# huawei-noah/Speech-Backbones

Hardware: AMD Instinct MI355X
Metric: mel-frames/sec at N=50 reverse-diffusion, 80x1024 batch (higher is better)
Workload: dtype f32 storage, f16 hi*hi MFMA + fp8 cross-term MFMA (3x3 Block convolutions, Upsample; bf16x3 elsewhere), f32 accumulate; 1 GPU; BASELINE config 2: Grad-TTS LJSpeech decoder, N=50, B=16/GPU synthetic 80x1024 mels, all-ones mask; per_gpu_batch=16, frames=1024, parallelism=utterance-shard x1, weights=seed-0 default init, Rezero.g=0.02, output_finite=True, conv_kernel=conv_ws.hip (persistent, wave-specialised), sub_batch_streams=0, hip_graph=False, launches_per_euler_step=64

## Files before the change

speech-backbones_amd/csrc/attn.hip:

```cpp
#include <cstring>
#include "common.h"
#include "kernels.h"

#ifndef GTTS_ATTN_HPW
#define GTTS_ATTN_HPW 2
#endif

namespace gtts {

struct AttnCtxArgs {
    const void *x;
    const unsigned char *wkv;
    float *partials;
    int C, HW, nstage, tiles, tps, nrec, nsplit, B;
    AttnTail tail;
};

__device__ __forceinline__ void pack8_split(const float (&v)[8], u32x4 &hi, u32x4 &lo) {
    bf16x8 vh, vl;
#pragma unroll
    for (int i = 0; i < 8; ++i) {
        __bf16 h, l;
        split_bf16(v[i], h, l);
        vh[i] = h;
        vl[i] = l;
    }
    hi = *reinterpret_cast<u32x4 *>(&vh);
    lo = *reinterpret_cast<u32x4 *>(&vl);
}

template <int NSPLIT, int FULLC, typename AT = float, int HPW = 1, int TAIL = 0>
__global__ __launch_bounds__(256 * HPW, HPW == 1 ? 2 : 1) void attn_ctx_kernel(const AttnCtxArgs a) {
    constexpr int AB = (int)sizeof(AT);
    static_assert(!TAIL || (FULLC && AB == 4), "the fused tail: whole 32-channel stages, fp32 storage");
    constexpr int KCH = ATTN_KCH, NKG = 2 * KCH;
    constexpr int NKGT = NKG / HPW;
    constexpr int WHEAD = 2 * NKG * 64;
    static_assert(HPW == 1 || HPW == 2, "one or two heads per workgroup");
    constexpr int SM16 = 2 * NKG * 256 + HPW * WHEAD;
    static_assert((size_t)SM16 * 16 >= (size_t)4 * HPW * ATTN_REC * 4, "merge records must fit the staging buffer");
    __shared__ __attribute__((aligned(16))) u32x4 s_all[SM16];
    u32x4 *s_ah = s_all, *s_al = s_all + NKG * 256;
    u32x4 *s_wall = s_all + 2 * NKG * 256;

    const int tid = threadIdx.x, lane = tid & 63;
    const int t255 = tid & 255, hw = __builtin_amdgcn_readfirstlane(tid >> 8);
    const int wave = (tid >> 6) & 3;
    const int l31 = lane & 31, kgl = lane >> 5;
    constexpr int HG = 4 / HPW;
    const int nsl = gridDim.x / (HG * a.B);
    const int wg = xcd_slot(blockIdx.x, gridDim.x);
    const int head = (wg % HG) * HPW + hw, slice = (wg / HG) % nsl, b = (wg / HG) / nsl;
    u32x4 *s_w = s_wall + hw * WHEAD;
    const int tile0 = slice * a.tps;
    const int tile1 = min(tile0 + a.tps, a.tiles);
    const AT *xb = reinterpret_cast<const AT *>(a.x) + (size_t)b * a.C * a.HW;
    const u32x4 *wblk = reinterpret_cast<const u32x4 *>(a.wkv) + (size_t)head * a.nstage * (2 * NKG * 64);

    float raw[NKGT][8];
    u32x4 wregs[KCH];
    const unsigned long long xaddr = reinterpret_cast<unsigned long long>(xb);
    const unsigned xlo = __builtin_amdgcn_readfirstlane((unsigned)xaddr);
    const unsigned xhi = __builtin_amdgcn_readfirstlane((unsigned)(xaddr >> 32));
    const int xbytes = a.C * a.HW * AB;
    const __amdgpu_buffer_rsrc_t rsx = __builtin_amdgcn_make_buffer_rsrc(
        reinterpret_cast<void *>(((unsigned long long)xhi << 32) | xlo), 0, __builtin_amdgcn_readfirstlane(xbytes), 0x00020000);
    [[maybe_unused]] float rawh[NKGT][8], tmask = 0.f;
    [[maybe_unused]] __amdgpu_buffer_rsrc_t rsh = rsx, rsi = rsx;
    [[maybe_unused]] const bool tail_store = (wg % HG) == 0;
    if constexpr (TAIL) {
        auto mk = [&](const void *p) {
            const unsigned long long u = reinterpret_cast<unsigned long long>(reinterpret_cast<const AT *>(p) + (size_t)b * a.C * a.HW);
            const unsigned lo = __builtin_amdgcn_readfirstlane((unsigned)u), hi = __builtin_amdgcn_readfirstlane((unsigned)(u >> 32));
            return __builtin_amdgcn_make_buffer_rsrc(reinterpret_cast<void *>(((unsigned long long)hi << 32) | lo), 0,
                                                     __builtin_amdgcn_readfirstlane(xbytes), 0x00020000);
        };
        rsh = mk(a.tail.h);
        rsi = mk(a.tail.xin);
    }
    auto apply_tail = [&](int tile, int stage) {
        if constexpr (TAIL) {
            const int n = tile * 256 + t255;
            const int voff = n < a.HW ? n * AB : xbytes;
#pragma unroll
            for (int kg = 0; kg < NKGT; ++kg) {
                const int cb = stage * 16 * KCH + (hw * NKGT + kg) * 8;
#pragma unroll
                for (int i = 0; i < 8; ++i) {
                    const float sc = a.tail.esc[(size_t)b * a.C + cb + i], sh = a.tail.esh[(size_t)b * a.C + cb + i];
                    const float v = tail_value(rawh[kg][i], raw[kg][i], sc, sh, tmask);
                    raw[kg][i] = v;
                    if (tail_store) __builtin_amdgcn_raw_buffer_store_b32(__builtin_bit_cast(int, v), rsx, voff, (cb + i) * a.HW * 4, GTTS_OUT_NT);
                }
            }
        }
    };
    auto load = [&](int tile, int stage) {
        const int n = tile * 256 + t255;
        const int voff = n < a.HW ? n * AB : xbytes;
        if constexpr (TAIL) {
            if (stage == 0) tmask = n < a.HW ? a.tail.mask[(size_t)b * a.tail.T + ((size_t)(n % a.tail.W) << a.tail.lvl)] : 0.f;
        }
#pragma unroll
        for (int kg = 0; kg < NKGT; ++kg) {
            const int cb = stage * 16 * KCH + (hw * NKGT + kg) * 8;
#pragma unroll
            for (int i = 0; i < 8; ++i) {
                const int c = FULLC ? cb + i : min(cb + i, a.C - 1);
                float v;
                if constexpr (TAIL) {
                    v = __builtin_bit_cast(float, __builtin_amdgcn_raw_buffer_load_b32(rsi, voff, c * a.HW * 4, 0));
                    rawh[kg][i] = __builtin_bit_cast(float, __builtin_amdgcn_raw_buffer_load_b32(rsh, voff, c * a.HW * 4, 0));
                } else if constexpr (AB == 4) v = __builtin_bit_cast(float, __builtin_amdgcn_raw_buffer_load_b32(rsx, voff, c * a.HW * 4, 0));
                else v = __builtin_bit_cast(float, (unsigned)(unsigned short)__builtin_amdgcn_raw_buffer_load_b16(rsx, voff, c * a.HW * 2, 0) << 16);
                raw[kg][i] = (FULLC || cb + i < a.C) ? v : 0.f;
            }
        }
        const u32x4 *g = wblk + (size_t)stage * (2 * NKG * 64);
#pragma unroll
        for (int j = 0; j < KCH; ++j) wregs[j] = g[t255 + j * 256];
    };

    const float NEG_INF = -__builtin_inff();
    float m_run = NEG_INF, z_run = 0.f;
    f32x16 ctx;
#pragma unroll
    for (int r = 0; r < 16; ++r) ctx[r] = 0.f;
    constexpr bool lo_on = NSPLIT > 1;

    load(tile0, 0);
    for (int tile = tile0; tile < tile1; ++tile) {
        f32x16 acc[2][2];
#pragma unroll
        for (int pf = 0; pf < 2; ++pf)
#pragma unroll
            for (int cf = 0; cf < 2; ++cf)
#pragma unroll
                for (int r = 0; r < 16; ++r) acc[pf][cf][r] = 0.f;

        for (int stage = 0; stage < a.nstage; ++stage) {
            apply_tail(tile, stage);
            lds_barrier();
#pragma unroll
            for (int kg = 0; kg < NKGT; ++kg) {
                u32x4 hi, lo;
                pack8_split(raw[kg], hi, lo);
                s_ah[(hw * NKGT + kg) * 256 + t255] = hi;
                s_al[(hw * NKGT + kg) * 256 + t255] = lo;
            }
#pragma unroll
            for (int j = 0; j < KCH; ++j) s_w[t255 + j * 256] = wregs[j];
            lds_barrier();
            if (stage + 1 < a.nstage) load(tile, stage + 1);
            else if (tile + 1 < tile1) load(tile + 1, 0);
#pragma unroll
            for (int kc = 0; kc < KCH; ++kc) {
                bf16x8 xh[2], xl[2], wh[2], wl[2];
#pragma unroll
                for (int pf = 0; pf < 2; ++pf) {
                    const int xi = (kc * 2 + kgl) * 256 + wave * 64 + pf * 32 + l31;
                    xh[pf] = *reinterpret_cast<const bf16x8 *>(&s_ah[xi]);
                    xl[pf] = *reinterpret_cast<const bf16x8 *>(&s_al[xi]);
                }
#pragma unroll
                for (int cf = 0; cf < 2; ++cf) {
                    const int wi = (kc * 2 + kgl) * 64 + cf * 32 + l31;
                    wh[cf] = *reinterpret_cast<const bf16x8 *>(&s_w[wi]);
                    wl[cf] = *reinterpret_cast<const bf16x8 *>(&s_w[wi + NKG * 64]);
                }
#pragma unroll
                for (int pf = 0; pf < 2; ++pf)
#pragma unroll
                    for (int cf = 0; cf < 2; ++cf) {
                        if (lo_on) {
                            acc[pf][cf] = __builtin_amdgcn_mfma_f32_32x32x16_bf16(xl[pf], wh[cf], acc[pf][cf], 0, 0, 0);
                            acc[pf][cf] = __builtin_amdgcn_mfma_f32_32x32x16_bf16(xh[pf], wl[cf], acc[pf][cf], 0, 0, 0);
                        }
                        acc[pf][cf] = __builtin_amdgcn_mfma_f32_32x32x16_bf16(xh[pf], wh[cf], acc[pf][cf], 0, 0, 0);
                    }
            }
        }

        const int nbase = tile * 256 + wave * 64 + 4 * kgl;
        const bool full = tile * 256 + 256 <= a.HW;
        float tmax = NEG_INF;
        if (full) {
#pragma unroll
            for (int pf = 0; pf < 2; ++pf)
#pragma unroll
                for (int rg = 0; rg < 16; ++rg) tmax = fmaxf(tmax, acc[pf][0][rg]);
        } else {
#pragma unroll
            for (int pf = 0; pf < 2; ++pf)
#pragma unroll
                for (int rg = 0; rg < 16; ++rg) {
                    const int n = nbase + pf * 32 + (rg & 3) + 8 * (rg >> 2);
                    if (n < a.HW) tmax = fmaxf(tmax, acc[pf][0][rg]);
                }
        }
        tmax = fmaxf(tmax, __shfl_xor(tmax, 32, 64));
        const float m_new = fmaxf(m_run, tmax);
        const float alpha = (m_run == NEG_INF) ? 0.f : __expf(m_run - m_new);
        const float msub = (m_new == NEG_INF) ? 0.f : m_new;
        constexpr float LOG2E = 1.44269504088896340736f;
        float psum = 0.f;
        if (full) {
#pragma unroll
            for (int pf = 0; pf < 2; ++pf)
#pragma unroll
                for (int rg = 0; rg < 16; ++rg) {
                    const float p = __builtin_amdgcn_exp2f((acc[pf][0][rg] - msub) * LOG2E);
                    acc[pf][0][rg] = p;
                    psum += p;
                }
        } else {
#pragma unroll
            for (int pf = 0; pf < 2; ++pf)
#pragma unroll
                for (int rg = 0; rg < 16; ++rg) {
                    const int n = nbase + pf * 32 + (rg & 3) + 8 * (rg >> 2);
                    const float p = (n < a.HW) ? __builtin_amdgcn_exp2f((acc[pf][0][rg] - msub) * LOG2E) : 0.f;
                    acc[pf][0][rg] = p;
                    psum += p;
                }
        }
        psum += __shfl_xor(psum, 32, 64);
        z_run = z_run * alpha + psum;
        m_run = m_new;
        if (__builtin_amdgcn_ballot_w64(alpha != 1.f) != 0ull) {
#pragma unroll
            for (int rg = 0; rg < 16; ++rg) {
                const int d = (rg & 3) + 8 * (rg >> 2) + 4 * kgl;
                ctx[rg] *= __shfl(alpha, d, 64);
            }
        }
#pragma unroll
        for (int pf = 0; pf < 2; ++pf)
#pragma unroll
            for (int hh = 0; hh < 2; ++hh) {
                float pv[8], vv[8];
#pragma unroll
                for (int i = 0; i < 8; ++i) {
                    pv[i] = acc[pf][0][hh * 8 + i];
                    vv[i] = acc[pf][1][hh * 8 + i];
                }
                u32x4 ph, pl, vh, vl;
                pack8_split(pv, ph, pl);
                pack8_split(vv, vh, vl);
                const bf16x8 Ph = *reinterpret_cast<bf16x8 *>(&ph), Pl = *reinterpret_cast<bf16x8 *>(&pl);
                const bf16x8 Vh = *reinterpret_cast<bf16x8 *>(&vh), Vl = *reinterpret_cast<bf16x8 *>(&vl);
                if (lo_on) {
                    ctx = __builtin_amdgcn_mfma_f32_32x32x16_bf16(Pl, Vh, ctx, 0, 0, 0);
                    ctx = __builtin_amdgcn_mfma_f32_32x32x16_bf16(Ph, Vl, ctx, 0, 0, 0);
                }
                ctx = __builtin_amdgcn_mfma_f32_32x32x16_bf16(Ph, Vh, ctx, 0, 0, 0);
            }
    }

    __syncthreads();
    float (*s_mrg)[ATTN_REC] = reinterpret_cast<float (*)[ATTN_REC]>(s_all) + hw * 4;
    {
        float *mine = s_mrg[wave];
        if (kgl == 0) {
            mine[l31] = m_run;
            mine[32 + l31] = z_run;
        }
#pragma unroll
        for (int rg = 0; rg < 16; ++rg) {
            const int d = (rg & 3) + 8 * (rg >> 2) + 4 * kgl;
            mine[64 + d * 32 + l31] = ctx[rg];
        }
    }
    __syncthreads();
    float *rec = a.partials + ((((size_t)b * 4 + head) * a.nrec) + (size_t)slice) * ATTN_REC;
#pragma unroll
    for (int k = 0; k < 4; ++k) {
        const int idx = t255 + 256 * k, d = idx >> 5;
        float M = NEG_INF;
#pragma unroll
        for (int w = 0; w < 4; ++w) M = fmaxf(M, s_mrg[w][d]);
        float acc_c = 0.f, acc_z = 0.f;
#pragma unroll
        for (int w = 0; w < 4; ++w) {
            const float mw = s_mrg[w][d];
            const float sc = (mw == NEG_INF) ? 0.f : __expf(mw - M);
            acc_c = fmaf(s_mrg[w][64 + idx], sc, acc_c);
            acc_z = fmaf(s_mrg[w][32 + d], sc, acc_z);
        }
        rec[64 + idx] = acc_c;
        if ((idx & 31) == 0) {
            rec[d] = M;
            rec[32 + d] = acc_z;
        }
    }
}

template <int NSPLIT, typename AT, int TAIL = 0>
__global__ __launch_bounds__(256, 2) void attn_ctx64_kernel(const AttnCtxArgs a) {
    constexpr int AB = (int)sizeof(AT);
    constexpr int C = 64, NKGT = C / 8;
    constexpr bool lo_on = NSPLIT > 1;
    __shared__ __attribute__((aligned(16))) u32x4 s_ah[NKGT * 64];
    __shared__ __attribute__((aligned(16))) u32x4 s_al[NKGT * 64];
    __shared__ __attribute__((aligned(16))) u32x4 s_w[4][1024];

    const int tid = threadIdx.x, lane = tid & 63;
    const int wave = __builtin_amdgcn_readfirstlane(tid >> 6);
    const int l31 = lane & 31, kgl = lane >> 5;
    const int nsl = gridDim.x / a.B;
    const int wg = xcd_slot(blockIdx.x, gridDim.x);
    const int slice = wg % nsl, b = wg / nsl;
    const int head = wave;
    const int tile0 = slice * a.tps, tile1 = min(tile0 + a.tps, a.tiles);
    const AT *xb = reinterpret_cast<const AT *>(a.x) + (size_t)b * C * a.HW;

    {
        const u32x4 *wsrc = reinterpret_cast<const u32x4 *>(a.wkv) + (size_t)head * 1024;
        u32x4 wr[16];
#pragma unroll
        for (int i = 0; i < 16; ++i) wr[i] = wsrc[lane + 64 * i];
#pragma unroll
        for (int i = 0; i < 16; ++i) s_w[wave][lane + 64 * i] = wr[i];
    }

    const unsigned long long xaddr = reinterpret_cast<unsigned long long>(xb);
    const unsigned xlo = __builtin_amdgcn_readfirstlane((unsigned)xaddr);
    const unsigned xhi = __builtin_amdgcn_readfirstlane((unsigned)(xaddr >> 32));
    const int xbytes = C * a.HW * AB;
    const __amdgpu_buffer_rsrc_t rsx = __builtin_amdgcn_make_buffer_rsrc(
        reinterpret_cast<void *>(((unsigned long long)xhi << 32) | xlo), 0, __builtin_amdgcn_readfirstlane(xbytes), 0x00020000);
    float raw[2][8];
    [[maybe_unused]] float rawh[2][8], tsc[2][8], tsh[2][8], tmask = 0.f;
    [[maybe_unused]] __amdgpu_buffer_rsrc_t rsh = rsx, rsi = rsx;
    if constexpr (TAIL) {
        static_assert(!TAIL || AB == 4, "the fused tail is the fp32-storage form");
        auto mk = [&](const void *p) {
            const unsigned long long u = reinterpret_cast<unsigned long long>(reinterpret_cast<const AT *>(p) + (size_t)b * C * a.HW);
            const unsigned lo = __builtin_amdgcn_readfirstlane((unsigned)u), hi = __builtin_amdgcn_readfirstlane((unsigned)(u >> 32));
            return __builtin_amdgcn_make_buffer_rsrc(reinterpret_cast<void *>(((unsigned long long)hi << 32) | lo), 0,
                                                     __builtin_amdgcn_readfirstlane(xbytes), 0x00020000);
        };
        rsh = mk(a.tail.h);
        rsi = mk(a.tail.xin);
#pragma unroll
        for (int it = 0; it < 2; ++it)
#pragma unroll
            for (int i = 0; i < 8; ++i) {
                const int c = (it * 4 + wave) * 8 + i;
                tsc[it][i] = a.tail.esc[(size_t)b * C + c];
                tsh[it][i] = a.tail.esh[(size_t)b * C + c];
            }
    }
    auto load = [&](int tile) {
        const int n = tile * 64 + lane;
        const int voff = n < a.HW ? n * AB : xbytes;
#pragma unroll
        for (int it = 0; it < 2; ++it)
#pragma unroll
            for (int i = 0; i < 8; ++i) {
                const int c = (it * 4 + wave) * 8 + i;
                if constexpr (TAIL) {
                    raw[it][i] = __builtin_bit_cast(float, __builtin_amdgcn_raw_buffer_load_b32(rsi, voff, c * a.HW * 4, 0));
                    rawh[it][i] = __builtin_bit_cast(float, __builtin_amdgcn_raw_buffer_load_b32(rsh, voff, c * a.HW * 4, 0));
                } else if constexpr (AB == 4) raw[it][i] = __builtin_bit_cast(float, __builtin_amdgcn_raw_buffer_load_b32(rsx, voff, c * a.HW * 4, 0));
                else raw[it][i] = __builtin_bit_cast(float, (unsigned)(unsigned short)__builtin_amdgcn_raw_buffer_load_b16(rsx, voff, c * a.HW * 2, 0) << 16);
            }
        if constexpr (TAIL) tmask = n < a.HW ? a.tail.mask[(size_t)b * a.tail.T + ((size_t)(n % a.tail.W) << a.tail.lvl)] : 0.f;
    };
    auto apply_tail = [&](int tile) {
        if constexpr (TAIL) {
            const int n = tile * 64 + lane;
            const int voff = n < a.HW ? n * AB : xbytes;
#pragma unroll
            for (int it = 0; it < 2; ++it)
#pragma unroll
                for (int i = 0; i < 8; ++i) {
                    const int c = (it * 4 + wave) * 8 + i;
                    const float v = tail_value(rawh[it][i], raw[it][i], tsc[it][i], tsh[it][i], tmask);
                    raw[it][i] = v;
                    __builtin_amdgcn_raw_buffer_store_b32(__builtin_bit_cast(int, v), rsx, voff, c * a.HW * 4, GTTS_OUT_NT);
                }
        }
    };

    const float NEG_INF = -__builtin_inff();
    float m_run = NEG_INF, z_run = 0.f;
    f32x16 ctx;
#pragma unroll
    for (int r = 0; r < 16; ++r) ctx[r] = 0.f;

    load(tile0);
    for (int tile = tile0; tile < tile1; ++tile) {
        apply_tail(tile);
        lds_barrier();
#pragma unroll
        for (int it = 0; it < 2; ++it) {
            u32x4 hi, lo;
            pack8_split(raw[it], hi, lo);
            s_ah[(it * 4 + wave) * 64 + lane] = hi;
            if (lo_on) s_al[(it * 4 + wave) * 64 + lane] = lo;
        }
        lds_barrier();
        load(min(tile + 1, tile1 - 1));

        f32x16 acc[2][2];
#pragma unroll
        for (int pf = 0; pf < 2; ++pf)
#pragma unroll
            for (int cf = 0; cf < 2; ++cf)
#pragma unroll
                for (int r = 0; r < 16; ++r) acc[pf][cf][r] = 0.f;
#pragma unroll
        for (int s = 0; s < 4; ++s) {
            bf16x8 xh[2], xl[2], wh[2], wl[2];
#pragma unroll
            for (int pf = 0; pf < 2; ++pf) {
                const int xi = (s * 2 + kgl) * 64 + pf * 32 + l31;
                xh[pf] = *reinterpret_cast<const bf16x8 *>(&s_ah[xi]);
                if (lo_on) xl[pf] = *reinterpret_cast<const bf16x8 *>(&s_al[xi]);
            }
#pragma unroll
            for (int cf = 0; cf < 2; ++cf) {
                const int wi = (s >> 1) * 512 + ((s & 1) * 2 + kgl) * 64 + cf * 32 + l31;
                wh[cf] = *reinterpret_cast<const bf16x8 *>(&s_w[wave][wi]);
                if (lo_on) wl[cf] = *reinterpret_cast<const bf16x8 *>(&s_w[wave][wi + 256]);
            }
#pragma unroll
            for (int pf = 0; pf < 2; ++pf)
#pragma unroll
                for (int cf = 0; cf < 2; ++cf) {
                    if (lo_on) {
                        acc[pf][cf] = __builtin_amdgcn_mfma_f32_32x32x16_bf16(xl[pf], wh[cf], acc[pf][cf], 0, 0, 0);
                        acc[pf][cf] = __builtin_amdgcn_mfma_f32_32x32x16_bf16(xh[pf], wl[cf], acc[pf][cf], 0, 0, 0);
                    }
                    acc[pf][cf] = __builtin_amdgcn_mfma_f32_32x32x16_bf16(xh[pf], wh[cf], acc[pf][cf], 0, 0, 0);
                }
        }

        const int nbase = tile * 64 + 4 * kgl;
        const bool full = tile * 64 + 64 <= a.HW;
        float tmax = NEG_INF;
        if (full) {
#pragma unroll
            for (int pf = 0; pf < 2; ++pf)
#pragma unroll
                for (int rg = 0; rg < 16; ++rg) tmax = fmaxf(tmax, acc[pf][0][rg]);
        } else {
#pragma unroll
            for (int pf = 0; pf < 2; ++pf)
#pragma unroll
                for (int rg = 0; rg < 16; ++rg) {
                    const int n = nbase + pf * 32 + (rg & 3) + 8 * (rg >> 2);
                    if (n < a.HW) tmax = fmaxf(tmax, acc[pf][0][rg]);
                }
        }
        tmax = fmaxf(tmax, __shfl_xor(tmax, 32, 64));
        const float m_new = fmaxf(m_run, tmax);
        const float alpha = (m_run == NEG_INF) ? 0.f : __expf(m_run - m_new);
        const float msub = (m_new == NEG_INF) ? 0.f : m_new;
        constexpr float LOG2E = 1.44269504088896340736f;
        float psum = 0.f;
        if (full) {
#pragma unroll
            for (int pf = 0; pf < 2; ++pf)
#pragma unroll
                for (int rg = 0; rg < 16; ++rg) {
                    const float p = __builtin_amdgcn_exp2f((acc[pf][0][rg] - msub) * LOG2E);
                    acc[pf][0][rg] = p;
                    psum += p;
                }
        } else {
#pragma unroll
            for (int pf = 0; pf < 2; ++pf)
#pragma unroll
                for (int rg = 0; rg < 16; ++rg) {
                    const int n = nbase + pf * 32 + (rg & 3) + 8 * (rg >> 2);
                    const float p = (n < a.HW) ? __builtin_amdgcn_exp2f((acc[pf][0][rg] - msub) * LOG2E) : 0.f;
                    acc[pf][0][rg] = p;
                    psum += p;
                }
        }
        psum += __shfl_xor(psum, 32, 64);
        z_run = z_run * alpha + psum;
        m_run = m_new;
        if (__builtin_amdgcn_ballot_w64(alpha != 1.f) != 0ull) {
#pragma unroll
            for (int rg = 0; rg < 16; ++rg) {
                const int d = (rg & 3) + 8 * (rg >> 2) + 4 * kgl;
                ctx[rg] *= __shfl(alpha, d, 64);
            }
        }
#pragma unroll
        for (int pf = 0; pf < 2; ++pf)
#pragma unroll
            for (int hh = 0; hh < 2; ++hh) {
                float pv[8], vv[8];
#pragma unroll
                for (int i = 0; i < 8; ++i) {
                    pv[i] = acc[pf][0][hh * 8 + i];
                    vv[i] = acc[pf][1][hh * 8 + i];
                }
                u32x4 ph, pl, vh, vl;
                pack8_split(pv, ph, pl);
                pack8_split(vv, vh, vl);
                const bf16x8 Ph = *reinterpret_cast<bf16x8 *>(&ph), Pl = *reinterpret_cast<bf16x8 *>(&pl);
                const bf16x8 Vh = *reinterpret_cast<bf16x8 *>(&vh), Vl = *reinterpret_cast<bf16x8 *>(&vl);
                if (lo_on) {
                    ctx = __builtin_amdgcn_mfma_f32_32x32x16_bf16(Pl, Vh, ctx, 0, 0, 0);
                    ctx = __builtin_amdgcn_mfma_f32_32x32x16_bf16(Ph, Vl, ctx, 0, 0, 0);
                }
                ctx = __builtin_amdgcn_mfma_f32_32x32x16_bf16(Ph, Vh, ctx, 0, 0, 0);
            }
    }

    float *rec = a.partials + ((((size_t)b * 4 + head) * a.nrec) + (size_t)slice) * ATTN_REC;
    if (kgl == 0) {
        rec[l31] = m_run;
        rec[32 + l31] = z_run;
    }
#pragma unroll
    for (int rg = 0; rg < 16; ++rg) {
        const int d = (rg & 3) + 8 * (rg >> 2) + 4 * kgl;
        rec[64 + d * 32 + l31] = ctx[rg];
    }
}

template <int NSPLIT, typename AT, int TAIL>
static hipError_t launch_ctx64(const AttnCtxArgs &a, dim3 grid, hipStream_t st, std::string *name) {
    if (name) return kernel_name(name, "gtts::attn_ctx64_kernel", NSPLIT, act_name<AT>(), TAIL);
    hipLaunchKernelGGL((attn_ctx64_kernel<NSPLIT, AT, TAIL>), grid, dim3(256), 0, st, a);
    return hipGetLastError();
}
template <int NSPLIT, int FULLC, typename AT, int TAIL>
static hipError_t launch_ctx(const AttnCtxArgs &a, int nslices, hipStream_t st, std::string *name) {
    constexpr int HPW = GTTS_ATTN_HPW;
    if (name) return kernel_name(name, "gtts::attn_ctx_kernel", NSPLIT, FULLC, act_name<AT>(), HPW, TAIL);
    hipLaunchKernelGGL((attn_ctx_kernel<NSPLIT, FULLC, AT, HPW, TAIL>), dim3(nslices * (4 / HPW) * a.B), dim3(256 * HPW), 0, st, a);
    return hipGetLastError();
}

hipError_t launch_attn_ctx(const void *x, const unsigned char *wkv, float *partials, int B, int C, int HW, int nsplit,
                           hipStream_t st, int act_bf16, const AttnTail *tail, std::string *name) {
    AttnGeom g = attn_geom(HW, C);
    if ((size_t)C * HW * 4 >= ((size_t)1 << 31)) return hipErrorInvalidValue;
    if (tail != nullptr && (C % 32 != 0 || act_bf16)) return hipErrorInvalidValue;
    if (act_bf16 && nsplit > 1) return hipErrorInvalidValue;
    AttnCtxArgs a;
    memset(&a, 0, sizeof(a));
    if (tail != nullptr) a.tail = *tail;
    a.x = x; a.wkv = wkv; a.partials = partials; a.C = C; a.HW = HW;
    a.nstage = (C + 16 * ATTN_KCH - 1) / (16 * ATTN_KCH);
    a.tiles = g.tiles; a.tps = g.tps; a.nrec = g.nrec; a.nsplit = nsplit; a.B = B;
    if (attn_head_per_wave(C)) {
        static_assert(ATTN_KCH == 2, "attn_ctx64_kernel indexes the packed k|v blocks as 32-channel stages");
        const dim3 grid64(g.nslices * B);
        if (act_bf16) return launch_ctx64<1, __bf16, 0>(a, grid64, st, name);
        if (tail != nullptr) return nsplit > 1 ? launch_ctx64<2, float, 1>(a, grid64, st, name) : launch_ctx64<1, float, 1>(a, grid64, st, name);
        return nsplit > 1 ? launch_ctx64<2, float, 0>(a, grid64, st, name) : launch_ctx64<1, float, 0>(a, grid64, st, name);
    }
    if (act_bf16) return C % 32 == 0 ? launch_ctx<1, 1, __bf16, 0>(a, g.nslices, st, name) : launch_ctx<1, 0, __bf16, 0>(a, g.nslices, st, name);
    if (tail != nullptr) return nsplit > 1 ? launch_ctx<2, 1, float, 1>(a, g.nslices, st, name) : launch_ctx<1, 1, float, 1>(a, g.nslices, st, name);
    if (C % 32 == 0) return nsplit > 1 ? launch_ctx<2, 1, float, 0>(a, g.nslices, st, name) : launch_ctx<1, 1, float, 0>(a, g.nslices, st, name);
    return nsplit > 1 ? launch_ctx<2, 0, float, 0>(a, g.nslices, st, name) : launch_ctx<1, 0, float, 0>(a, g.nslices, st, name);
}

__global__ __launch_bounds__(1024) void attn_merge_kernel(const float *__restrict__ partials, float *__restrict__ ctxn,
                                                           int nrec) {
    extern __shared__ float sm[];
    float *s_w = sm;
    float *s_red = sm + (size_t)nrec * 32;
    float *s_M = s_red + 1024;
    float *s_Zi = s_M + 32;
    const int head = blockIdx.x, b = blockIdx.y, tid = threadIdx.x;
    const int d = tid & 31, g = tid >> 5;
    const float *rec = partials + ((size_t)b * 4 + head) * nrec * ATTN_REC;
    const float NEG_INF = -__builtin_inff();
    float mx = NEG_INF;
    for (int i = g; i < nrec; i += 32) mx = fmaxf(mx, rec[(size_t)i * ATTN_REC + d]);
    s_red[g * 32 + d] = mx;
    __syncthreads();
    if (g == 0) {
        float M = NEG_INF;
        for (int k = 0; k < 32; ++k) M = fmaxf(M, s_red[k * 32 + d]);
        s_M[d] = M;
    }
    __syncthreads();
    const float M = s_M[d];
    float zz = 0.f;
    for (int i = g; i < nrec; i += 32) {
        const float mi = rec[(size_t)i * ATTN_REC + d];
        const float w = (mi == NEG_INF) ? 0.f : expf(mi - M);
        s_w[i * 32 + d] = w;
        zz += rec[(size_t)i * ATTN_REC + 32 + d] * w;
    }
    __syncthreads();
    s_red[g * 32 + d] = zz;
    __syncthreads();
    if (g == 0) {
        float Z = 0.f;
        for (int k = 0; k < 32; ++k) Z += s_red[k * 32 + d];
        s_Zi[d] = 1.0f / Z;
    }
    __syncthreads();
    const int dd = tid >> 5;
    float acc = 0.f;
    const float *cp = rec + 64 + tid;
    int i = 0;
    for (; i + 4 <= nrec; i += 4) {
        const float c0 = cp[(size_t)(i + 0) * ATTN_REC], c1 = cp[(size_t)(i + 1) * ATTN_REC];
        const float c2 = cp[(size_t)(i + 2) * ATTN_REC], c3 = cp[(size_t)(i + 3) * ATTN_REC];
        acc = fmaf(c0, s_w[(i + 0) * 32 + dd], acc);
        acc = fmaf(c1, s_w[(i + 1) * 32 + dd], acc);
        acc = fmaf(c2, s_w[(i + 2) * 32 + dd], acc);
        acc = fmaf(c3, s_w[(i + 3) * 32 + dd], acc);
    }
    for (; i < nrec; ++i) acc = fmaf(cp[(size_t)i * ATTN_REC], s_w[i * 32 + dd], acc);
    ctxn[(((size_t)b * 4 + head) * 1024) + tid] = acc * s_Zi[dd];
}

hipError_t launch_attn_merge(const float *partials, float *ctxn, int B, int nrec, hipStream_t st) {
    const size_t smem = ((size_t)nrec * 32 + 1024 + 64) * sizeof(float);
    if (smem > 160 * 1024) return hipErrorInvalidValue;
    if (smem > 48 * 1024) {
        hipError_t e = hipFuncSetAttribute(reinterpret_cast<const void *>(&attn_merge_kernel),
                                           hipFuncAttributeMaxDynamicSharedMemorySize, (int)smem);
        if (e != hipSuccess) return e;
    }
    hipLaunchKernelGGL(attn_merge_kernel, dim3(4, B), dim3(1024), smem, st, partials, ctxn, nrec);
    return hipGetLastError();
}

constexpr int FOLD_CO = 8;
struct AttnFoldArgs {
    const float *ctxn, *wq, *wout, *bout, *g;
    unsigned char *wpk;
    size_t wpk_bstride;
    float *biasb;
    int C, MT, nkg;
    int ndn;
    const float *dn_w, *dn_wo, *dn_vw;
    unsigned char *dn_wpk;
    size_t dn_bstride;
    float *dn_btab;
    int dn_MT, dn_nkg;
};
__global__ __launch_bounds__(256) void attn_fold_kernel(const AttnFoldArgs a) {
    __shared__ float s_U[FOLD_CO][128];
    __shared__ float s_part[4][FOLD_CO][128];
    const int co0 = blockIdx.x * FOLD_CO, b = blockIdx.z, tid = threadIdx.x;
    const int C = a.C;
    const int tap = (int)blockIdx.y < a.ndn ? (int)blockIdx.y : -1;
    const float *wout = tap >= 0 ? a.dn_wo + (size_t)tap * C * 128 : a.wout;
    const float *cb = a.ctxn + (size_t)b * 4096;
    {
        const int j = tid & 127, h = j >> 5, d = j & 31;
        const float4 *cx = reinterpret_cast<const float4 *>(cb + (h * 32 + d) * 32);
        float4 cv[8];
#pragma unroll
        for (int e = 0; e < 8; ++e) cv[e] = cx[e];
#pragma unroll
        for (int rr = 0; rr < FOLD_CO / 2; ++rr) {
            const int r = (tid >> 7) * (FOLD_CO / 2) + rr;
            const float4 *wo = reinterpret_cast<const float4 *>(wout + (size_t)(co0 + r) * 128 + h * 32);
            float acc = 0.f;
#pragma unroll
            for (int e = 0; e < 8; ++e) {
                const float4 w4 = wo[e];
                acc = fmaf(w4.x, cv[e].x, acc); acc = fmaf(w4.y, cv[e].y, acc);
                acc = fmaf(w4.z, cv[e].z, acc); acc = fmaf(w4.w, cv[e].w, acc);
            }
            s_U[r][j] = acc;
        }
    }
    __syncthreads();
    const float gv = a.g[0];
    const int MT = tap >= 0 ? a.dn_MT : a.MT, nkg = tap >= 0 ? a.dn_nkg : a.nkg;
    const int ncot = (C + MT - 1) / MT;
    __bf16 *wp = tap >= 0 ? reinterpret_cast<__bf16 *>(a.dn_wpk + (size_t)b * a.dn_bstride)
                          : reinterpret_cast<__bf16 *>(a.wpk + (size_t)b * a.wpk_bstride);
    const int ky = tap >= 0 ? tap / 3 : 0, kx = tap >= 0 ? tap - 3 * ky : 0;
    const int nst = tap >= 0 ? 3 : 1, tps = nst;
    const int Cc = C < 256 ? C : 256;
    const int nj = 256 / Cc >= 4 ? 4 : (256 / Cc >= 2 ? 2 : 1);
    const int jq = tid / Cc, cl = tid - jq * Cc;
    const int jn = 128 / nj;
    const bool active = jq < nj;
    for (int ci = cl; ci < C; ci += Cc) {
        float acc[FOLD_CO];
#pragma unroll
        for (int r = 0; r < FOLD_CO; ++r) acc[r] = 0.f;
        const float *qp = a.wq + (size_t)(active ? jq * jn : 0) * C + ci;
        for (int j0 = 0; j0 < (active ? jn : 0); j0 += 8) {
            float q[8];
#pragma unroll
            for (int u = 0; u < 8; ++u) q[u] = qp[(size_t)(j0 + u) * C];
#pragma unroll
            for (int u = 0; u < 8; ++u)
#pragma unroll
                for (int r = 0; r < FOLD_CO; ++r) acc[r] = fmaf(s_U[r][jq * jn + j0 + u], q[u], acc[r]);
        }
        if (nj > 1) {
            if (active && jq > 0) {
#pragma unroll
                for (int r = 0; r < FOLD_CO; ++r) s_part[jq][r][cl] = acc[r];
            }
            __syncthreads();
            if (jq == 0) {
                for (int k = 1; k < nj; ++k)
#pragma unroll
                    for (int r = 0; r < FOLD_CO; ++r) acc[r] += s_part[k][r][cl];
            }
        }
        if (jq == 0) {
            const int chunk = ci / (8 * nkg), kg = (ci >> 3) % nkg, i = ci & 7;
#pragma unroll
            for (int r = 0; r < FOLD_CO; ++r) {
                const int co = co0 + r, cot = co / MT, m = co % MT;
                const size_t blk = ((size_t)chunk * nst + ky) * ncot + cot;
                const size_t blk_elems = (size_t)tps * MT * 16 * nkg;
                const size_t e_hi = blk * blk_elems + ((size_t)((0 * tps + kx) * nkg + kg) * MT + m) * 8 + i;
                const size_t e_lo = blk * blk_elems + ((size_t)((1 * tps + kx) * nkg + kg) * MT + m) * 8 + i;
                const float v = tap >= 0 ? fmaf(acc[r], gv, a.dn_w[((size_t)co * C + ci) * 9 + tap]) : acc[r] * gv;
                __bf16 hi, lo;
                split_bf16(v, hi, lo);
                wp[e_hi] = hi;
                wp[e_lo] = lo;
            }
        }
    }
    if (tap < 0 && tid < FOLD_CO) a.biasb[(size_t)b * C + co0 + tid] = gv * a.bout[co0 + tid];
    if (tap == 0 && tid < FOLD_CO) {
        const int co = co0 + tid;
        float *t = a.dn_btab + (size_t)b * 6 * C + co;
#pragma unroll
        for (int k = 0; k < 3; ++k) {
            const float v0 = a.dn_vw[(size_t)(0 + k) * C + co], v1 = a.dn_vw[(size_t)(3 + k) * C + co], v2 = a.dn_vw[(size_t)(6 + k) * C + co];
            t[(size_t)(0 + k) * C] = gv * (v1 + v2);
            t[(size_t)(3 + k) * C] = gv * ((v0 + v1) + v2);
        }
    }
}

hipError_t launch_attn_fold(const float *ctxn, const float *wq, const float *wout, const float *bout, const float *g,
                            unsigned char *wpk, size_t wpk_bstride, float *biasb, int B, int C, hipStream_t st,
                            const AttnFoldDn *dn) {
    if (C % 16 != 0) return hipErrorInvalidValue;
    ConvGeom geom = conv_geom(CONV_P1, C, C);
    if (C % (16 * geom.kch) != 0) return hipErrorInvalidValue;
    if (wpk == nullptr && dn == nullptr) return hipErrorInvalidValue;
    AttnFoldArgs a;
    memset(&a, 0, sizeof(a));
    a.ctxn = ctxn; a.wq = wq; a.wout = wout; a.bout = bout; a.g = g;
    a.wpk = wpk; a.wpk_bstride = wpk_bstride; a.biasb = biasb;
    a.C = C; a.MT = geom.MT; a.nkg = 2 * geom.kch;
    if (dn != nullptr) {
        ConvGeom gd = conv_geom(CONV_DN, C, C);
        if (C % (16 * gd.kch) != 0 || C % gd.MT != 0 || gd.nst != 3 || gd.tps != 3) return hipErrorInvalidValue;
        if (dn->bstride < conv_packed_bytes(CONV_DN, C, C)) return hipErrorInvalidValue;
        a.ndn = 9;
        a.dn_w = dn->w; a.dn_wo = dn->wo; a.dn_vw = dn->vw;
        a.dn_wpk = dn->wpk; a.dn_bstride = dn->bstride; a.dn_btab = dn->btab;
        a.dn_MT = gd.MT; a.dn_nkg = 2 * gd.kch;
    }
    hipLaunchKernelGGL(attn_fold_kernel, dim3(C / FOLD_CO, a.ndn + (wpk != nullptr ? 1 : 0), B), dim3(256), 0, st, a);
    return hipGetLastError();
}

__global__ __launch_bounds__(128) void attn_dn_precompose_kernel(const float *__restrict__ w, const float *__restrict__ wout,
                                                                  const float *__restrict__ bout, float *__restrict__ wo,
                                                                  float *__restrict__ vw, int C) {
    const int co = blockIdx.x, tap = blockIdx.y, j = threadIdx.x;
    const float *wr = w + (size_t)co * C * 9 + tap;
    float acc = 0.f, accb = 0.f;
    for (int c = 0; c < C; ++c) {
        const float wv = wr[(size_t)c * 9];
        acc = fmaf(wv, wout[(size_t)c * 128 + j], acc);
        accb = fmaf(wv, bout[c], accb);
    }
    wo[((size_t)tap * C + co) * 128 + j] = acc;
    if (j == 0) vw[(size_t)tap * C + co] = accb;
}

hipError_t launch_attn_dn_precompose(const float *w, const float *wout, const float *bout, float *wo, float *vw, int C, hipStream_t st) {
    hipLaunchKernelGGL(attn_dn_precompose_kernel, dim3(C, 9), dim3(128), 0, st, w, wout, bout, wo, vw, C);
    return hipGetLastError();
}

}
```

Baseline: 53200 mel-frames/s.

## Double-buffer attention context staging with paired-pixel vector loads

Reworks both attention context kernels so each thread loads two adjacent pixels per channel with 64-bit buffer loads and stores. It also rotates two register sets, and in the main kernel two LDS staging buffers, so the next stage's global loads are issued before the current MFMA work and one barrier per step is dropped. The tail scale/shift loads move to a lane shuffle and the mask goes through a buffer resource. This adds register and LDS pressure, which may reduce occupancy, and HW must now be even.

```diff
diff --git a/speech-backbones_amd/csrc/attn.hip b/speech-backbones_amd/csrc/attn.hip
--- a/speech-backbones_amd/csrc/attn.hip
+++ b/speech-backbones_amd/csrc/attn.hip
@@ -4,6 +4,9 @@
 
 #ifndef GTTS_ATTN_HPW
 #define GTTS_ATTN_HPW 2
+#endif
+#ifndef GTTS_ATTN_NBUF
+#define GTTS_ATTN_NBUF 2
 #endif
 
 namespace gtts {
@@ -15,6 +18,24 @@
     int C, HW, nstage, tiles, tps, nrec, nsplit, B;
     AttnTail tail;
 };
+
+__device__ __forceinline__ float u2f(unsigned u) { return __builtin_bit_cast(float, u); }
+typedef float f32x2 __attribute__((ext_vector_type(2)));
+typedef unsigned u32x2 __attribute__((ext_vector_type(2)));
+__device__ __forceinline__ f32x2 load_pair_f32(__amdgpu_buffer_rsrc_t rs, int voff, int soff) {
+    return __builtin_bit_cast(f32x2, __builtin_amdgcn_raw_buffer_load_b64(rs, voff, soff, 0));
+}
+__device__ __forceinline__ f32x2 load_pair_bf16(__amdgpu_buffer_rsrc_t rs, int voff, int soff) {
+    const unsigned v = __builtin_amdgcn_raw_buffer_load_b32(rs, voff, soff, 0);
+    f32x2 r;
+    r.x = u2f(v << 16);
+    r.y = u2f(v & 0xffff0000u);
+    return r;
+}
+__device__ __forceinline__ void consume_here(f32x2 &v) { asm volatile("" : "+v"(v)); }
+__device__ __forceinline__ void store_pair_f32(f32x2 v, __amdgpu_buffer_rsrc_t rs, int voff, int soff) {
+    __builtin_amdgcn_raw_buffer_store_b64(__builtin_bit_cast(u32x2, v), rs, voff, soff, GTTS_OUT_NT);
+}
 
 __device__ __forceinline__ void pack8_split(const float (&v)[8], u32x4 &hi, u32x4 &lo) {
     bf16x8 vh, vl;
@@ -37,11 +58,11 @@
     constexpr int NKGT = NKG / HPW;
     constexpr int WHEAD = 2 * NKG * 64;
     static_assert(HPW == 1 || HPW == 2, "one or two heads per workgroup");
+    constexpr int NBUF = GTTS_ATTN_NBUF;
+    static_assert(NBUF == 1 || NBUF == 2, "one staging buffer, or two in rotation");
     constexpr int SM16 = 2 * NKG * 256 + HPW * WHEAD;
     static_assert((size_t)SM16 * 16 >= (size_t)4 * HPW * ATTN_REC * 4, "merge records must fit the staging buffer");
-    __shared__ __attribute__((aligned(16))) u32x4 s_all[SM16];
-    u32x4 *s_ah = s_all, *s_al = s_all + NKG * 256;
-    u32x4 *s_wall = s_all + 2 * NKG * 256;
+    __shared__ __attribute__((aligned(16))) u32x4 s_all[NBUF * SM16];
 
     const int tid = threadIdx.x, lane = tid & 63;
     const int t255 = tid & 255, hw = __builtin_amdgcn_readfirstlane(tid >> 8);
@@ -51,22 +72,24 @@
     const int nsl = gridDim.x / (HG * a.B);
     const int wg = xcd_slot(blockIdx.x, gridDim.x);
     const int head = (wg % HG) * HPW + hw, slice = (wg / HG) % nsl, b = (wg / HG) / nsl;
-    u32x4 *s_w = s_wall + hw * WHEAD;
     const int tile0 = slice * a.tps;
     const int tile1 = min(tile0 + a.tps, a.tiles);
     const AT *xb = reinterpret_cast<const AT *>(a.x) + (size_t)b * a.C * a.HW;
     const u32x4 *wblk = reinterpret_cast<const u32x4 *>(a.wkv) + (size_t)head * a.nstage * (2 * NKG * 64);
 
-    float raw[NKGT][8];
-    u32x4 wregs[KCH];
+    static_assert(NKGT % 2 == 0, "whole pixel-pair items per thread");
+    constexpr int NIT = NKGT / 2;
+    const int pr = tid & 127, kgw = __builtin_amdgcn_readfirstlane(tid >> 7);
+    f32x2 rawA[NIT][8], rawB[NIT][8];
+    u32x4 wregsA[KCH], wregsB[KCH];
     const unsigned long long xaddr = reinterpret_cast<unsigned long long>(xb);
     const unsigned xlo = __builtin_amdgcn_readfirstlane((unsigned)xaddr);
     const unsigned xhi = __builtin_amdgcn_readfirstlane((unsigned)(xaddr >> 32));
     const int xbytes = a.C * a.HW * AB;
     const __amdgpu_buffer_rsrc_t rsx = __builtin_amdgcn_make_buffer_rsrc(
         reinterpret_cast<void *>(((unsigned long long)xhi << 32) | xlo), 0, __builtin_amdgcn_readfirstlane(xbytes), 0x00020000);
-    [[maybe_unused]] float rawh[NKGT][8], tmask = 0.f;
-    [[maybe_unused]] __amdgpu_buffer_rsrc_t rsh = rsx, rsi = rsx;
+    [[maybe_unused]] f32x2 rawhA[NIT][8], rawhB[NIT][8], tmA = {0.f, 0.f}, tmB = {0.f, 0.f};
+    [[maybe_unused]] __amdgpu_buffer_rsrc_t rsh = rsx, rsi = rsx, rsm = rsx;
     [[maybe_unused]] const bool tail_store = (wg % HG) == 0;
     if constexpr (TAIL) {
         auto mk = [&](const void *p) {
@@ -77,48 +100,68 @@
         };
         rsh = mk(a.tail.h);
         rsi = mk(a.tail.xin);
-    }
-    auto apply_tail = [&](int tile, int stage) {
+        const unsigned long long um = reinterpret_cast<unsigned long long>(a.tail.mask + (size_t)b * a.tail.T);
+        rsm = __builtin_amdgcn_make_buffer_rsrc(reinterpret_cast<void *>(((unsigned long long)__builtin_amdgcn_readfirstlane((unsigned)(um >> 32)) << 32) |
+                                                                       (unsigned)__builtin_amdgcn_readfirstlane((unsigned)um)),
+                                                0, __builtin_amdgcn_readfirstlane(a.tail.T * 4), 0x00020000);
+    }
+    auto trim = [&](int stage, f32x2 (&rx)[NIT][8], f32x2 (&rh)[NIT][8]) {
+#pragma unroll
+        for (int it = 0; it < NIT; ++it)
+#pragma unroll
+            for (int i = 0; i < 8; ++i) {
+                consume_here(rx[it][i]);
+                if constexpr (TAIL) consume_here(rh[it][i]);
+                if (!FULLC && stage * 16 * KCH + (it * 2 * HPW + kgw) * 8 + i >= a.C) rx[it][i] = f32x2{0.f, 0.f};
+            }
+    };
+    auto apply_tail = [&](int tile, int stage, f32x2 (&rx)[NIT][8], f32x2 (&rh)[NIT][8], f32x2 &rm) {
+        trim(stage, rx, rh);
         if constexpr (TAIL) {
-            const int n = tile * 256 + t255;
+            const int n = tile * 256 + 2 * pr;
             const int voff = n < a.HW ? n * AB : xbytes;
 #pragma unroll
-            for (int kg = 0; kg < NKGT; ++kg) {
-                const int cb = stage * 16 * KCH + (hw * NKGT + kg) * 8;
+            for (int it = 0; it < NIT; ++it) {
+                const int cb = stage * 16 * KCH + (it * 2 * HPW + kgw) * 8;
 #pragma unroll
                 for (int i = 0; i < 8; ++i) {
                     const float sc = a.tail.esc[(size_t)b * a.C + cb + i], sh = a.tail.esh[(size_t)b * a.C + cb + i];
-                    const float v = tail_value(rawh[kg][i], raw[kg][i], sc, sh, tmask);
-                    raw[kg][i] = v;
-                    if (tail_store) __builtin_amdgcn_raw_buffer_store_b32(__builtin_bit_cast(int, v), rsx, voff, (cb + i) * a.HW * 4, GTTS_OUT_NT);
+                    f32x2 v;
+                    v.x = tail_value(rh[it][i].x, rx[it][i].x, sc, sh, rm.x);
+                    v.y = tail_value(rh[it][i].y, rx[it][i].y, sc, sh, rm.y);
+                    rx[it][i] = v;
+                }
+                if (tail_store) {
+#pragma unroll
+                    for (int i = 0; i < 8; ++i) store_pair_f32(rx[it][i], rsx, voff, (cb + i) * a.HW * 4);
                 }
             }
         }
     };
-    auto load = [&](int tile, int stage) {
-        const int n = tile * 256 + t255;
+    auto load = [&](int tile, int stage, f32x2 (&rx)[NIT][8], f32x2 (&rh)[NIT][8], f32x2 &rm, u32x4 (&wr)[KCH]) {
+        const int n = tile * 256 + 2 * pr;
         const int voff = n < a.HW ? n * AB : xbytes;
-        if constexpr (TAIL) {
-            if (stage == 0) tmask = n < a.HW ? a.tail.mask[(size_t)b * a.tail.T + ((size_t)(n % a.tail.W) << a.tail.lvl)] : 0.f;
-        }
-#pragma unroll
-        for (int kg = 0; kg < NKGT; ++kg) {
-            const int cb = stage * 16 * KCH + (hw * NKGT + kg) * 8;
+#pragma unroll
+        for (int it = 0; it < NIT; ++it) {
+            const int cb = stage * 16 * KCH + (it * 2 * HPW + kgw) * 8;
 #pragma unroll
             for (int i = 0; i < 8; ++i) {
                 const int c = FULLC ? cb + i : min(cb + i, a.C - 1);
-                float v;
+                const int so = c * a.HW * AB;
                 if constexpr (TAIL) {
-                    v = __builtin_bit_cast(float, __builtin_amdgcn_raw_buffer_load_b32(rsi, voff, c * a.HW * 4, 0));
-                    rawh[kg][i] = __builtin_bit_cast(float, __builtin_amdgcn_raw_buffer_load_b32(rsh, voff, c * a.HW * 4, 0));
-                } else if constexpr (AB == 4) v = __builtin_bit_cast(float, __builtin_amdgcn_raw_buffer_load_b32(rsx, voff, c * a.HW * 4, 0));
-                else v = __builtin_bit_cast(float, (unsigned)(unsigned short)__builtin_amdgcn_raw_buffer_load_b16(rsx, voff, c * a.HW * 2, 0) << 16);
-                raw[kg][i] = (FULLC || cb + i < a.C) ? v : 0.f;
-            }
+                    rx[it][i] = load_pair_f32(rsi, voff, so);
+                    rh[it][i] = load_pair_f32(rsh, voff, so);
+                } else if constexpr (AB == 4) rx[it][i] = load_pair_f32(rsx, voff, so);
+                else rx[it][i] = load_pair_bf16(rsx, voff, so);
+            }
+        }
+        if constexpr (TAIL) {
+            rm.x = u2f(__builtin_amdgcn_raw_buffer_load_b32(rsm, n < a.HW ? ((n % a.tail.W) << a.tail.lvl) * 4 : a.tail.T * 4, 0, 0));
+            rm.y = u2f(__builtin_amdgcn_raw_buffer_load_b32(rsm, n + 1 < a.HW ? (((n + 1) % a.tail.W) << a.tail.lvl) * 4 : a.tail.T * 4, 0, 0));
         }
         const u32x4 *g = wblk + (size_t)stage * (2 * NKG * 64);
 #pragma unroll
-        for (int j = 0; j < KCH; ++j) wregs[j] = g[t255 + j * 256];
+        for (int j = 0; j < KCH; ++j) wr[j] = g[t255 + j * 256];
     };
 
     const float NEG_INF = -__builtin_inff();
@@ -127,60 +170,9 @@
 #pragma unroll
     for (int r = 0; r < 16; ++r) ctx[r] = 0.f;
     constexpr bool lo_on = NSPLIT > 1;
-
-    load(tile0, 0);
-    for (int tile = tile0; tile < tile1; ++tile) {
-        f32x16 acc[2][2];
-#pragma unroll
-        for (int pf = 0; pf < 2; ++pf)
-#pragma unroll
-            for (int cf = 0; cf < 2; ++cf)
-#pragma unroll
-                for (int r = 0; r < 16; ++r) acc[pf][cf][r] = 0.f;
-
-        for (int stage = 0; stage < a.nstage; ++stage) {
-            apply_tail(tile, stage);
-            lds_barrier();
-#pragma unroll
-            for (int kg = 0; kg < NKGT; ++kg) {
-                u32x4 hi, lo;
-                pack8_split(raw[kg], hi, lo);
-                s_ah[(hw * NKGT + kg) * 256 + t255] = hi;
-                s_al[(hw * NKGT + kg) * 256 + t255] = lo;
-            }
-#pragma unroll
-            for (int j = 0; j < KCH; ++j) s_w[t255 + j * 256] = wregs[j];
-            lds_barrier();
-            if (stage + 1 < a.nstage) load(tile, stage + 1);
-            else if (tile + 1 < tile1) load(tile + 1, 0);
-#pragma unroll
-            for (int kc = 0; kc < KCH; ++kc) {
-                bf16x8 xh[2], xl[2], wh[2], wl[2];
-#pragma unroll
-                for (int pf = 0; pf < 2; ++pf) {
-                    const int xi = (kc * 2 + kgl) * 256 + wave * 64 + pf * 32 + l31;
-                    xh[pf] = *reinterpret_cast<const bf16x8 *>(&s_ah[xi]);
-                    xl[pf] = *reinterpret_cast<const bf16x8 *>(&s_al[xi]);
-                }
-#pragma unroll
-                for (int cf = 0; cf < 2; ++cf) {
-                    const int wi = (kc * 2 + kgl) * 64 + cf * 32 + l31;
-                    wh[cf] = *reinterpret_cast<const bf16x8 *>(&s_w[wi]);
-                    wl[cf] = *reinterpret_cast<const bf16x8 *>(&s_w[wi + NKG * 64]);
-                }
-#pragma unroll
-                for (int pf = 0; pf < 2; ++pf)
-#pragma unroll
-                    for (int cf = 0; cf < 2; ++cf) {
-                        if (lo_on) {
-                            acc[pf][cf] = __builtin_amdgcn_mfma_f32_32x32x16_bf16(xl[pf], wh[cf], acc[pf][cf], 0, 0, 0);
-                            acc[pf][cf] = __builtin_amdgcn_mfma_f32_32x32x16_bf16(xh[pf], wl[cf], acc[pf][cf], 0, 0, 0);
-                        }
-                        acc[pf][cf] = __builtin_amdgcn_mfma_f32_32x32x16_bf16(xh[pf], wh[cf], acc[pf][cf], 0, 0, 0);
-                    }
-            }
-        }
-
+    f32x16 acc[2][2];
+
+    auto finish_tile = [&](int tile) {
         const int nbase = tile * 256 + wave * 64 + 4 * kgl;
         const bool full = tile * 256 + 256 <= a.HW;
         float tmax = NEG_INF;
@@ -255,6 +247,82 @@
                 }
                 ctx = __builtin_amdgcn_mfma_f32_32x32x16_bf16(Ph, Vh, ctx, 0, 0, 0);
             }
+    };
+    auto step = [&](int tile, int stage, int ptile, int pstage, int buf, f32x2 (&rx)[NIT][8], f32x2 (&rh)[NIT][8], f32x2 &rm,
+                    u32x4 (&wr)[KCH]) {
+        u32x4 *s_ah = s_all + buf * SM16, *s_al = s_ah + NKG * 256;
+        u32x4 *s_w = s_ah + 2 * NKG * 256 + hw * WHEAD;
+        if (stage == 0) {
+#pragma unroll
+            for (int pf = 0; pf < 2; ++pf)
+#pragma unroll
+                for (int cf = 0; cf < 2; ++cf)
+#pragma unroll
+                    for (int r = 0; r < 16; ++r) acc[pf][cf][r] = 0.f;
+        }
+        apply_tail(tile, stage, rx, rh, rm);
+        if (NBUF == 1) lds_barrier();
+#pragma unroll
+        for (int it = 0; it < NIT; ++it)
+#pragma unroll
+            for (int px = 0; px < 2; ++px) {
+                float v[8];
+#pragma unroll
+                for (int i = 0; i < 8; ++i) v[i] = px ? rx[it][i].y : rx[it][i].x;
+                u32x4 hi, lo;
+                pack8_split(v, hi, lo);
+                s_ah[(it * 2 * HPW + kgw) * 256 + 2 * pr + px] = hi;
+                s_al[(it * 2 * HPW + kgw) * 256 + 2 * pr + px] = lo;
+            }
+#pragma unroll
+        for (int j = 0; j < KCH; ++j) s_w[t255 + j * 256] = wr[j];
+        load(ptile, pstage, rx, rh, rm, wr);
+        lds_barrier();
+#pragma unroll
+        for (int kc = 0; kc < KCH; ++kc) {
+            bf16x8 xh[2], xl[2], wh[2], wl[2];
+#pragma unroll
+            for (int pf = 0; pf < 2; ++pf) {
+                const int xi = (kc * 2 + kgl) * 256 + wave * 64 + pf * 32 + l31;
+                xh[pf] = *reinterpret_cast<const bf16x8 *>(&s_ah[xi]);
+                xl[pf] = *reinterpret_cast<const bf16x8 *>(&s_al[xi]);
+            }
+#pragma unroll
+            for (int cf = 0; cf < 2; ++cf) {
+                const int wi = (kc * 2 + kgl) * 64 + cf * 32 + l31;
+                wh[cf] = *reinterpret_cast<const bf16x8 *>(&s_w[wi]);
+                wl[cf] = *reinterpret_cast<const bf16x8 *>(&s_w[wi + NKG * 64]);
+            }
+#pragma unroll
+            for (int pf = 0; pf < 2; ++pf)
+#pragma unroll
+                for (int cf = 0; cf < 2; ++cf) {
+                    if (lo_on) {
+                        acc[pf][cf] = __builtin_amdgcn_mfma_f32_32x32x16_bf16(xl[pf], wh[cf], acc[pf][cf], 0, 0, 0);
+                        acc[pf][cf] = __builtin_amdgcn_mfma_f32_32x32x16_bf16(xh[pf], wl[cf], acc[pf][cf], 0, 0, 0);
+                    }
+                    acc[pf][cf] = __builtin_amdgcn_mfma_f32_32x32x16_bf16(xh[pf], wh[cf], acc[pf][cf], 0, 0, 0);
+                }
+        }
+        if (stage == a.nstage - 1) finish_tile(tile);
+    };
+    if (tile0 < tile1) {
+        const int ns = a.nstage;
+        int tile = tile0, stage = 0, pt = tile0, ps = 0;
+        auto next = [&](int &t, int &st) { if (++st == ns) { st = 0; ++t; } };
+        load(pt, ps, rawA, rawhA, tmA, wregsA);
+        next(pt, ps);
+        __builtin_amdgcn_sched_barrier(0);
+        load(pt < tile1 ? pt : tile1 - 1, pt < tile1 ? ps : ns - 1, rawB, rawhB, tmB, wregsB);
+        next(pt, ps);
+        int left = (tile1 - tile0) * ns;
+        for (; left >= 2; left -= 2) {
+            step(tile, stage, pt < tile1 ? pt : tile1 - 1, pt < tile1 ? ps : ns - 1, 0, rawA, rawhA, tmA, wregsA);
+            next(tile, stage); next(pt, ps);
+            step(tile, stage, pt < tile1 ? pt : tile1 - 1, pt < tile1 ? ps : ns - 1, NBUF - 1, rawB, rawhB, tmB, wregsB);
+            next(tile, stage); next(pt, ps);
+        }
+        if (left) step(tile, stage, tile, stage, 0, rawA, rawhA, tmA, wregsA);
     }
 
     __syncthreads();
@@ -329,9 +397,12 @@
     const int xbytes = C * a.HW * AB;
     const __amdgpu_buffer_rsrc_t rsx = __builtin_amdgcn_make_buffer_rsrc(
         reinterpret_cast<void *>(((unsigned long long)xhi << 32) | xlo), 0, __builtin_amdgcn_readfirstlane(xbytes), 0x00020000);
-    float raw[2][8];
-    [[maybe_unused]] float rawh[2][8], tsc[2][8], tsh[2][8], tmask = 0.f;
-    [[maybe_unused]] __amdgpu_buffer_rsrc_t rsh = rsx, rsi = rsx;
+    const int kgt = wave * 2 + kgl;
+    const int prow = kgl * 8 * a.HW * AB;
+    f32x2 rawA[8], rawB[8];
+    [[maybe_unused]] f32x2 rawhA[8], rawhB[8], tmA = {0.f, 0.f}, tmB = {0.f, 0.f};
+    [[maybe_unused]] float tsc = 0.f, tsh = 0.f;
+    [[maybe_unused]] __amdgpu_buffer_rsrc_t rsh = rsx, rsi = rsx, rsm = rsx;
     if constexpr (TAIL) {
         static_assert(!TAIL || AB == 4, "the fused tail is the fp32-storage form");
         auto mk = [&](const void *p) {
@@ -342,44 +413,50 @@
         };
         rsh = mk(a.tail.h);
         rsi = mk(a.tail.xin);
-#pragma unroll
-        for (int it = 0; it < 2; ++it)
+        const unsigned long long um = reinterpret_cast<unsigned long long>(a.tail.mask + (size_t)b * a.tail.T);
+        rsm = __builtin_amdgcn_make_buffer_rsrc(reinterpret_cast<void *>(((unsigned long long)__builtin_amdgcn_readfirstlane((unsigned)(um >> 32)) << 32) |
+                                                                       (unsigned)__builtin_amdgcn_readfirstlane((unsigned)um)),
+                                                0, __builtin_amdgcn_readfirstlane(a.tail.T * 4), 0x00020000);
+        tsc = a.tail.esc[(size_t)b * C + lane];
+        tsh = a.tail.esh[(size_t)b * C + lane];
+    }
+    auto load = [&](int tile, f32x2 (&rx)[8], f32x2 (&rh)[8], f32x2 &rm) {
+        const int n = tile * 64 + 2 * l31;
+        const int voff = n < a.HW ? n * AB + prow : xbytes;
+#pragma unroll
+        for (int i = 0; i < 8; ++i) {
+            const int so = (wave * 16 + i) * a.HW * AB;
+            if constexpr (TAIL) {
+                rx[i] = load_pair_f32(rsi, voff, so);
+                rh[i] = load_pair_f32(rsh, voff, so);
+            } else if constexpr (AB == 4) rx[i] = load_pair_f32(rsx, voff, so);
+            else rx[i] = load_pair_bf16(rsx, voff, so);
+        }
+        if constexpr (TAIL) {
+            rm.x = u2f(__builtin_amdgcn_raw_buffer_load_b32(rsm, n < a.HW ? ((n % a.tail.W) << a.tail.lvl) * 4 : a.tail.T * 4, 0, 0));
+            rm.y = u2f(__builtin_amdgcn_raw_buffer_load_b32(rsm, n + 1 < a.HW ? (((n + 1) % a.tail.W) << a.tail.lvl) * 4 : a.tail.T * 4, 0, 0));
+        }
+    };
+    auto apply_tail = [&](int tile, f32x2 (&rx)[8], f32x2 (&rh)[8], f32x2 &rm) {
+#pragma unroll
+        for (int i = 0; i < 8; ++i) {
+            consume_here(rx[i]);
+            if constexpr (TAIL) consume_here(rh[i]);
+        }
+        if constexpr (TAIL) {
+            const int n = tile * 64 + 2 * l31;
+            const int voff = n < a.HW ? n * AB + prow : xbytes;
+            asm volatile("" : "+v"(tsc), "+v"(tsh));
 #pragma unroll
             for (int i = 0; i < 8; ++i) {
-                const int c = (it * 4 + wave) * 8 + i;
-                tsc[it][i] = a.tail.esc[(size_t)b * C + c];
-                tsh[it][i] = a.tail.esh[(size_t)b * C + c];
-            }
-    }
-    auto load = [&](int tile) {
-        const int n = tile * 64 + lane;
-        const int voff = n < a.HW ? n * AB : xbytes;
-#pragma unroll
-        for (int it = 0; it < 2; ++it)
-#pragma unroll
-            for (int i = 0; i < 8; ++i) {
-                const int c = (it * 4 + wave) * 8 + i;
-                if constexpr (TAIL) {
-                    raw[it][i] = __builtin_bit_cast(float, __builtin_amdgcn_raw_buffer_load_b32(rsi, voff, c * a.HW * 4, 0));
-                    rawh[it][i] = __builtin_bit_cast(float, __builtin_amdgcn_raw_buffer_load_b32(rsh, voff, c * a.HW * 4, 0));
-                } else if constexpr (AB == 4) raw[it][i] = __builtin_bit_cast(float, __builtin_amdgcn_raw_buffer_load_b32(rsx, voff, c * a.HW * 4, 0));
-                else raw[it][i] = __builtin_bit_cast(float, (unsigned)(unsigned short)__builtin_amdgcn_raw_buffer_load_b16(rsx, voff, c * a.HW * 2, 0) << 16);
-            }
-        if constexpr (TAIL) tmask = n < a.HW ? a.tail.mask[(size_t)b * a.tail.T + ((size_t)(n % a.tail.W) << a.tail.lvl)] : 0.f;
-    };
-    auto apply_tail = [&](int tile) {
-        if constexpr (TAIL) {
-            const int n = tile * 64 + lane;
-            const int voff = n < a.HW ? n * AB : xbytes;
-#pragma unroll
-            for (int it = 0; it < 2; ++it)
-#pragma unroll
-                for (int i = 0; i < 8; ++i) {
-                    const int c = (it * 4 + wave) * 8 + i;
-                    const float v = tail_value(rawh[it][i], raw[it][i], tsc[it][i], tsh[it][i], tmask);
-                    raw[it][i] = v;
-                    __builtin_amdgcn_raw_buffer_store_b32(__builtin_bit_cast(int, v), rsx, voff, c * a.HW * 4, GTTS_OUT_NT);
-                }
+                const float sc = __shfl(tsc, kgt * 8 + i, 64), sh = __shfl(tsh, kgt * 8 + i, 64);
+                f32x2 v;
+                v.x = tail_value(rh[i].x, rx[i].x, sc, sh, rm.x);
+                v.y = tail_value(rh[i].y, rx[i].y, sc, sh, rm.y);
+                rx[i] = v;
+            }
+#pragma unroll
+            for (int i = 0; i < 8; ++i) store_pair_f32(rx[i], rsx, voff, (wave * 16 + i) * a.HW * 4);
         }
     };
 
@@ -389,19 +466,20 @@
 #pragma unroll
     for (int r = 0; r < 16; ++r) ctx[r] = 0.f;
 
-    load(tile0);
-    for (int tile = tile0; tile < tile1; ++tile) {
-        apply_tail(tile);
+    auto step = [&](int tile, int pf, f32x2 (&rx)[8], f32x2 (&rh)[8], f32x2 &rm) {
+        apply_tail(tile, rx, rh, rm);
         lds_barrier();
 #pragma unroll
-        for (int it = 0; it < 2; ++it) {
+        for (int px = 0; px < 2; ++px) {
+            float v[8];
+#pragma unroll
+            for (int i = 0; i < 8; ++i) v[i] = px ? rx[i].y : rx[i].x;
             u32x4 hi, lo;
-            pack8_split(raw[it], hi, lo);
-            s_ah[(it * 4 + wave) * 64 + lane] = hi;
-            if (lo_on) s_al[(it * 4 + wave) * 64 + lane] = lo;
+            pack8_split(v, hi, lo);
+            s_ah[kgt * 64 + 2 * l31 + px] = hi;
+            if (lo_on) s_al[kgt * 64 + 2 * l31 + px] = lo;
         }
         lds_barrier();
-        load(min(tile + 1, tile1 - 1));
 
         f32x16 acc[2][2];
 #pragma unroll
@@ -436,6 +514,8 @@
                     acc[pf][cf] = __builtin_amdgcn_mfma_f32_32x32x16_bf16(xh[pf], wh[cf], acc[pf][cf], 0, 0, 0);
                 }
         }
+
+        load(pf, rx, rh, rm);
 
         const int nbase = tile * 64 + 4 * kgl;
         const bool full = tile * 64 + 64 <= a.HW;
@@ -511,17 +591,29 @@
                 }
                 ctx = __builtin_amdgcn_mfma_f32_32x32x16_bf16(Ph, Vh, ctx, 0, 0, 0);
             }
-    }
-
+    };
+    if (tile0 < tile1) {
+        load(tile0, rawA, rawhA, tmA);
+        __builtin_amdgcn_sched_barrier(0);
+        load(min(tile0 + 1, tile1 - 1), rawB, rawhB, tmB);
+        int tile = tile0;
+        for (; tile + 1 < tile1; tile += 2) {
+            step(tile, min(tile + 2, tile1 - 1), rawA, rawhA, tmA);
+            step(tile + 1, min(tile + 3, tile1 - 1), rawB, rawhB, tmB);
+        }
+        if (tile < tile1) step(tile, tile, rawA, rawhA, tmA);
+    }
+
+    const int lane_e = __builtin_amdgcn_mbcnt_hi(~0u, __builtin_amdgcn_mbcnt_lo(~0u, 0u)), l31e = lane_e & 31, kgle = lane_e >> 5;
     float *rec = a.partials + ((((size_t)b * 4 + head) * a.nrec) + (size_t)slice) * ATTN_REC;
-    if (kgl == 0) {
-        rec[l31] = m_run;
-        rec[32 + l31] = z_run;
+    if (kgle == 0) {
+        rec[l31e] = m_run;
+        rec[32 + l31e] = z_run;
     }
 #pragma unroll
     for (int rg = 0; rg < 16; ++rg) {
-        const int d = (rg & 3) + 8 * (rg >> 2) + 4 * kgl;
-        rec[64 + d * 32 + l31] = ctx[rg];
+        const int d = (rg & 3) + 8 * (rg >> 2) + 4 * kgle;
+        rec[64 + d * 32 + l31e] = ctx[rg];
     }
 }
 
@@ -544,6 +636,7 @@
     AttnGeom g = attn_geom(HW, C);
     if ((size_t)C * HW * 4 >= ((size_t)1 << 31)) return hipErrorInvalidValue;
     if (tail != nullptr && (C % 32 != 0 || act_bf16)) return hipErrorInvalidValue;
+    if (HW & 1) return hipErrorInvalidValue;
     if (act_bf16 && nsplit > 1) return hipErrorInvalidValue;
     AttnCtxArgs a;
     memset(&a, 0, sizeof(a));
```

New measurement: 53130 mel-frames/s. No clear change (-0.1%).
